# t0m1ab/alphazero

Measured on AMD Instinct MI355X. Metric: self-play games/sec (whole node), Othello 8x8 @100 sims/move, higher is better.
Workload: dtype f32; 1 GPU; BASELINE configs[1] literal: Othello 8x8, 4096 concurrent games/GPU, 100 sims/move, 1 MI355X; concurrent_games_per_gpu=4096, sims_per_move=100, parallelism=game-sharded x1, dense_layers=float32 fma chains on the f32-input MFMA

## Files before the change

### alphazero_amd/csrc/az_net.hip

```cpp
#include <math.h>
#include <stdlib.h>
#include <string.h>

#include <map>
#include <string>
#include <vector>

#include "az_device.h"
#include <hip/hip_ext.h>
#include "az_host.h"

typedef float f32x4 __attribute__((ext_vector_type(4)));
#define MFMA(a, b, c) __builtin_amdgcn_mfma_f32_16x16x4f32((a), (b), (c), 0, 0, 0)
typedef float f32x16 __attribute__((ext_vector_type(16)));
typedef float f32x2 __attribute__((ext_vector_type(2)));
#define MFMA32(a, b, c) __builtin_amdgcn_mfma_f32_32x32x2f32((a), (b), (c), 0, 0, 0)

#define NCH 32
#define PLANE_STRIDE(x) (((x) + 1) | 1)

#ifdef AZ_PROBE
__device__ unsigned long long az_probe_buf[8192 * 8];
#define STAMP(var) { __builtin_amdgcn_sched_barrier(0); var = __builtin_amdgcn_s_memtime(); asm volatile("s_waitcnt lgkmcnt(0)" ::: "memory"); __builtin_amdgcn_sched_barrier(0); }
#else
// ... 1316 lines not shown
        ST_A(0, sa0, as_) ST_A(1, sa1, as_) ST_A(2, sa2, as_) ST_A(3, sa3, as_)           \
        ST_B(0, sb0, bs_) ST_B(1, sb1, bs_) ST_B(2, sb2, bs_) ST_B(3, sb3, bs_)           \
    }
#define FRD 4
#define GEMM_COMPUTE(buf)                                                                 \
    {                                                                                     \
        const float *as = As + (buf) * BM * ASTR + (wm0 + (lane & 31)) * ASTR + (lane >> 5);   \
        const float *bs = Bs + (buf) * BK * BSTR + (lane >> 5) * BSTR + wn0 + (lane & 31);     \
        float afr[FRD][TM], bfr[FRD][TN];                                                 \
        _Pragma("unroll") for (int p = 0; p < FRD - 1; ++p) {                             \
            _Pragma("unroll") for (int tm = 0; tm < TM; ++tm) afr[p][tm] = as[tm * 32 * ASTR + p * 2];          \
            _Pragma("unroll") for (int tn = 0; tn < TN; ++tn) bfr[p][tn] = bs[p * 2 * BSTR + tn * 32];          \
        }                                                                                 \
        _Pragma("unroll") for (int ks = 0; ks < BK / 2; ++ks) {                           \
            if (ks + FRD - 1 < BK / 2) {                                                  \
                _Pragma("unroll") for (int tm = 0; tm < TM; ++tm) afr[(ks + FRD - 1) % FRD][tm] = as[tm * 32 * ASTR + (ks + FRD - 1) * 2];   \
                _Pragma("unroll") for (int tn = 0; tn < TN; ++tn) bfr[(ks + FRD - 1) % FRD][tn] = bs[(ks + FRD - 1) * 2 * BSTR + tn * 32];   \
            }                                                                             \
            __builtin_amdgcn_sched_barrier(0);                                            \
            _Pragma("unroll") for (int tm = 0; tm < TM; ++tm)                             \
                _Pragma("unroll") for (int tn = 0; tn < TN; ++tn) acc[tm][tn] = MFMA32(afr[ks % FRD][tm], bfr[ks % FRD][tn], acc[tm][tn]); \
            __builtin_amdgcn_sched_barrier(0);                                            \
        }                                                                                 \
    }
    static_assert(A_LD <= 4 && B_LD <= 4, "staging register budget");
    const int T = KT > 0 ? KT : K / BK;
    GEMM_ISSUE_R(0)
    if (T > 1) GEMM_ISSUE_S(BK)
    GEMM_STORE_R(0)
    __syncthreads();
    unsigned long long p0 = 0, p1 = 0, p2 = 0, p3 = 0, p4 = 0, ph_issue = 0, ph_comp = 0, ph_store = 0, ph_bar = 0, p_begin = 0;
    (void)p0; (void)p1; (void)p2; (void)p3; (void)p4; (void)ph_issue; (void)ph_comp; (void)ph_store; (void)ph_bar; (void)p_begin;
    STAMP(p_begin)
#ifdef AZ_PROBE
    const unsigned long long rt_begin = __builtin_amdgcn_s_memrealtime();
#endif
#define GEMM_PAIR(t)                                                                      \
    {                                                                                     \
        STAMP(p0)                                                                         \
        if ((t) + 2 < T) GEMM_ISSUE_R(((t) + 2) * BK)                                     \
        STAMP(p1)                                                                         \
        GEMM_COMPUTE(0)                                                                   \
        STAMP(p2)                                                                         \
        if ((t) + 1 < T) GEMM_STORE_S(1)                                                  \
        STAMP(p3)                                                                         \
        __syncthreads();                                                                  \
        STAMP(p4)                                                                         \
        ph_issue += p1 - p0; ph_comp += p2 - p1; ph_store += p3 - p2; ph_bar += p4 - p3;  \
        if ((t) + 1 < T) {                                                                \
            STAMP(p0)                                                                     \
            if ((t) + 3 < T) GEMM_ISSUE_S(((t) + 3) * BK)                                 \
            STAMP(p1)                                                                     \
            GEMM_COMPUTE(1)                                                               \
            STAMP(p2)                                                                     \
            if ((t) + 2 < T) GEMM_STORE_R(0)                                              \
            STAMP(p3)                                                                     \
            __syncthreads();                                                              \
            STAMP(p4)                                                                     \
            ph_issue += p1 - p0; ph_comp += p2 - p1; ph_store += p3 - p2; ph_bar += p4 - p3;  \
        }                                                                                 \
    }
    if constexpr (KT > 0) {
#pragma unroll
        for (int t = 0; t < KT; t += 2) GEMM_PAIR(t)
    } else {
        for (int t = 0; t < T; t += 2) GEMM_PAIR(t)
    }
#undef GEMM_PAIR
#undef GEMM_ISSUE_R
#undef GEMM_ISSUE_S
#undef GEMM_STORE_R
#undef GEMM_STORE_S
#undef GEMM_COMPUTE
#undef FRD
#undef LD_A
#undef LD_B
#undef ST_A
#undef ST_B
#ifdef AZ_PROBE
    if (tid == 0 && bid < 8192) {
        unsigned long long p_end = 0;
        STAMP(p_end)
        unsigned long long *o = az_probe_buf + (size_t)bid * 8;
        o[0] = ph_issue; o[1] = ph_comp; o[2] = ph_store; o[3] = ph_bar; o[4] = p_end - p_begin; o[5] = p_begin; o[6] = p_end;
        o[7] = __builtin_amdgcn_s_memrealtime() - rt_begin;
    }
#endif
#pragma unroll
    for (int tm = 0; tm < TM; ++tm)
#pragma unroll
        for (int tn = 0; tn < TN; ++tn)
#pragma unroll
            for (int r = 0; r < 16; ++r) {
                int row = bm0 + wm0 + tm * 32 + (r & 3) + 8 * (r >> 2) + 4 * (lane >> 5);
                int col = bn0 + wn0 + tn * 32 + (lane & 31);
                float v = acc[tm][tn][r];
                if (RELU) v = v > 0.0f ? v : 0.0f;
                if (row < M) C[(size_t)row * N + col] = v;
            }
}

template <bool RELU>
__global__ __launch_bounds__(256) __attribute__((amdgpu_waves_per_eu(1, 1))) void k_gemm_solo(const float *__restrict__ A, const float *__restrict__ Bw,
                                                                                           const float *__restrict__ bias, float *__restrict__ C, int M, int N,
                                                                                           int K, const int *__restrict__ dyn_count) {
    if (dyn_count) { int c = *dyn_count; M = c < M ? c : M; }
    constexpr int BM = 256, BN = 256, BK = 32, ASTR = BK + 1, BSTR = BN;
    const int nbx = N / BN, nb = nbx * (int)gridDim.y;
    int bid = (int)blockIdx.y * nbx + (int)blockIdx.x;
    if (nb % 8 == 0) bid = (bid % 8) * (nb / 8) + bid / 8;
    const int tile_y = bid / nbx, tile_x = bid % nbx;
    int tme = 4;
    if ((M + 63) / 64 <= (int)gridDim.y) tme = 1;
    else if ((M + 127) / 128 <= (int)gridDim.y) tme = 2;
    const int BMe = 64 * tme;
    if (tile_y * BMe >= M) return;
#ifdef AZ_PROBE
    unsigned long long pk0, pk1, pl0, pl1;
    const unsigned long long rt0 = __builtin_amdgcn_s_memrealtime();
    STAMP(pk0)
#endif
    extern __shared__ __attribute__((aligned(16))) float gsm[];
    float *As = gsm;
    float *Bs = gsm + 2 * BM * ASTR;
    const int tid = threadIdx.x, wave = tid >> 6, lane = tid & 63;
    const int wm0 = (wave >> 1) * 32 * tme, wn0 = (wave & 1) * 128;
    const int bm0 = tile_y * BMe, bn0 = tile_x * BN;
    f32x16 acc[4][4];
    {
        const float one = lane < 32 ? 1.0f : 0.0f;
#pragma unroll
        for (int tn = 0; tn < 4; ++tn) {
            const float bv = lane < 32 ? bias[bn0 + wn0 + tn * 32 + lane] : 0.0f;
#pragma unroll
            for (int tm = 0; tm < 4; ++tm) {
                f32x16 z;
#pragma unroll
                for (int r = 0; r < 16; ++r) z[r] = 0.0f;
                acc[tm][tn] = MFMA32(one, bv, z);
            }
        }
    }
    const int arow = tid >> 3, aq = tid & 7;
    unsigned aoff0, aoff1, aoff2, aoff3, aoff4, aoff5, aoff6, aoff7;
#define SOLO_AOFF(i)                                                       \
    {                                                                      \
        int gr = bm0 + arow + 32 * i;                                      \
        gr = gr < M ? gr : M - 1;                                          \
        aoff##i = (unsigned)(((size_t)gr * K + 4 * aq) * sizeof(float));   \
    }
    SOLO_AOFF(0) SOLO_AOFF(1) SOLO_AOFF(2) SOLO_AOFF(3) SOLO_AOFF(4) SOLO_AOFF(5) SOLO_AOFF(6) SOLO_AOFF(7)
    const unsigned boff = (unsigned)(((size_t)(tid >> 6) * N + 4 * (tid & 63)) * sizeof(float));
    const float *Bt = Bw + bn0;
    float4 ra0, ra1, ra2, ra3, ra4, ra5, ra6, ra7, rb0, rb1, rb2, rb3, rb4, rb5, rb6, rb7;
#define SOLO_LDA(i, k0) ra##i = *reinterpret_cast<const float4 *>(reinterpret_cast<const char *>(A + (k0)) + aoff##i);
#define SOLO_LDB(i, k0) rb##i = *reinterpret_cast<const float4 *>(reinterpret_cast<const char *>(Bt + (size_t)((k0) + 4 * i) * N) + boff);
#define SOLO_LD(i, k0) { SOLO_LDA(i, k0) SOLO_LDB(i, k0) }
#define SOLO_ISSUE(k0) SOLO_LD(0, k0) SOLO_LD(1, k0) SOLO_LD(2, k0) SOLO_LD(3, k0) SOLO_LD(4, k0) SOLO_LD(5, k0) SOLO_LD(6, k0) SOLO_LD(7, k0)
#define SOLO_STA(i, as_)                       \
    {                                          \
        float *d = (as_) + 32 * i * ASTR;      \
        d[0] = ra##i.x;                        \
        d[1] = ra##i.y;                        \
        d[2] = ra##i.z;                        \
        d[3] = ra##i.w;                        \
    }
#define SOLO_STB(i, bs_) *reinterpret_cast<float4 *>((bs_) + 4 * i * BSTR) = rb##i;
#define SOLO_ST(i) { SOLO_STA(i, as_) SOLO_STB(i, bs_) }
#define SOLO_STASH(buf)                                                                                                      \
    {                                                                                                                        \
        float *as_ = As + (buf) * BM * ASTR + arow * ASTR + 4 * aq, *bs_ = Bs + (buf) * BK * BSTR + (tid >> 6) * BSTR + 4 * (tid & 63); \
        SOLO_ST(0) SOLO_ST(1) SOLO_ST(2) SOLO_ST(3) SOLO_ST(4) SOLO_ST(5) SOLO_ST(6) SOLO_ST(7)                              \
    }
#define SOLO_FENCE() { __builtin_amdgcn_sched_barrier(0); asm volatile("" ::: "memory"); __builtin_amdgcn_sched_barrier(0); }
#define SOLO_COMPUTE(buf, NEXT, k0n, TME)                                                                            \
    {                                                                                                            \
        const float *as = As + (buf) * BM * ASTR + (wm0 + (lane & 31)) * ASTR + (lane >> 5);                     \
        const float *bs = Bs + (buf) * BK * BSTR + (lane >> 5) * BSTR + wn0 + (lane & 31);                       \
        float *as_ = As + ((buf) ^ 1) * BM * ASTR + arow * ASTR + 4 * aq, *bs_ = Bs + ((buf) ^ 1) * BK * BSTR + (tid >> 6) * BSTR + 4 * (tid & 63); \
        float afr[2][4], bfr[2][4];                                                                              \
        _Pragma("unroll") for (int x = 0; x < 4; ++x) { if (x < TME) afr[0][x] = as[x * 32 * ASTR]; bfr[0][x] = bs[x * 32]; } \
        _Pragma("unroll") for (int ks = 0; ks < BK / 2; ++ks) {                                                  \
// ... 233 lines not shown
        for (int i = 0; i < 16; ++i) acc = fmaf(x[k0 + i], wa[i], acc);
        if (k0 + 32 < K) {
#pragma unroll
            for (int i = 0; i < 16; ++i) wa[i] = w[(size_t)(k0 + 32 + i) * N];
        }
#pragma unroll
        for (int i = 0; i < 16; ++i) acc = fmaf(x[k0 + 16 + i], wb[i], acc);
    }
    if (RELU) acc = acc > 0.0f ? acc : 0.0f;
    if (n < N) Y[(size_t)m * N + n] = acc;
}

template <bool RELU, int NT>
__global__ __launch_bounds__(64 * NT) void k_dense_frag(const float *__restrict__ X, const float *__restrict__ Wq, const float *__restrict__ bias,
                                                        float *__restrict__ Y, int M, int N, int K, const int *__restrict__ dyn_count) {
    if (dyn_count) { int c = *dyn_count; M = c < M ? c : M; }
    constexpr int NTHR = 64 * NT, PF = 8;
    const int brow0 = blockIdx.y * 16;
    if (brow0 >= M) return;
    extern __shared__ __attribute__((aligned(16))) float dfs[];
    const int XSTR = K + 4, NKB = K / 16, NTILES = N / 16;
    const int tid = threadIdx.x, wave = tid >> 6, lane = tid & 63;
    const int m = lane & 15, kq = lane >> 4;
    const int ct = blockIdx.x * NT + wave;
    const float4 *wq = reinterpret_cast<const float4 *>(Wq) + (size_t)ct * 64 + lane;
    const size_t wstep = (size_t)NTILES * 64;
    float4 bq[PF];
#pragma unroll
    for (int p = 0; p < PF; ++p) bq[p] = wq[(size_t)p * wstep];
    const float bv = bias[ct * 16 + m];
    {
        const int kv = K / 4, rows = (M - brow0) < 16 ? (M - brow0) : 16, nv = rows * kv;
        for (int q0 = 0; q0 < nv; q0 += 4 * NTHR) {
            float4 rx[4];
#pragma unroll
            for (int i = 0; i < 4; ++i) {
                const int q = q0 + tid + NTHR * i;
                rx[i] = make_float4(0, 0, 0, 0);
                if (q < nv) rx[i] = reinterpret_cast<const float4 *>(X + (size_t)(brow0 + q / kv) * K)[q % kv];
            }
#pragma unroll
            for (int i = 0; i < 4; ++i) {
                const int q = q0 + tid + NTHR * i;
                if (q < nv) *reinterpret_cast<float4 *>(dfs + (q / kv) * XSTR + 4 * (q % kv)) = rx[i];
            }
        }
    }
    __syncthreads();
    f32x4 acc = (f32x4){bv, bv, bv, bv};
    const float *xa = dfs + m * XSTR + kq;
    for (int kb0 = 0; kb0 < NKB; kb0 += PF) {
#pragma unroll
        for (int p = 0; p < PF; ++p) {
            const int kb = kb0 + p;
            const float4 b = bq[p];
            if (kb + PF < NKB) bq[p] = wq[(size_t)(kb + PF) * wstep];
            const float a0 = xa[16 * kb], a1 = xa[16 * kb + 4], a2 = xa[16 * kb + 8], a3 = xa[16 * kb + 12];
            __builtin_amdgcn_sched_barrier(0);
            acc = MFMA(a0, b.x, acc);
            acc = MFMA(a1, b.y, acc);
            acc = MFMA(a2, b.z, acc);
            acc = MFMA(a3, b.w, acc);
            __builtin_amdgcn_sched_barrier(0);
        }
    }
#pragma unroll
    for (int r = 0; r < 4; ++r) {
        const int row = brow0 + 4 * kq + r;
        float v = acc[r];
        if (RELU) v = v > 0.0f ? v : 0.0f;
        if (row < M) Y[(size_t)row * N + ct * 16 + m] = v;
    }
}

__global__ void k_retile_q(const float *__restrict__ W, float *__restrict__ dst, int K, int N) {
    const int i = blockIdx.x * blockDim.x + threadIdx.x;
    if (i >= K * N) return;
    const int ii = i % 4, lane = (i / 4) % 64, NTL = N / 16, nt = (i / 256) % NTL, kb = i / (256 * NTL);
    dst[i] = W[(size_t)(16 * kb + 4 * ii + (lane >> 4)) * N + 16 * nt + (lane & 15)];
}

template <int BM, int BN>
constexpr int gemm_lds_bytes() { return 4 * (2 * BM * (32 + 1) + 2 * 32 * BN); }

template <int NT>
__global__ __launch_bounds__(256) void k_heads(const float *__restrict__ X, const float *__restrict__ Wh,
                                               const float *__restrict__ bh, int M, int K, int A,
                                               float *__restrict__ probs, float *__restrict__ value, const int *__restrict__ dyn_count) {
    if (dyn_count) { int c = *dyn_count; M = c < M ? c : M; }
    if ((int)blockIdx.x * 32 >= M) return;
    constexpr int NH = NT * 16, KC = 128, XSTR = KC + 2, WSTR = NH, NS = (NT + 1) / 2;
    constexpr int X_LD = 32 * KC / 4 / 256, W_LD = (KC * NH / 4 + 255) / 256;
    static_assert(X_LD == 4 && W_LD <= 10, "staging registers");
    extern __shared__ __attribute__((aligned(16))) float hsm[];
    float *Xs = hsm;
    float *Ws = Xs + 32 * XSTR;
    float *Ls = Ws + KC * WSTR;
    float *rsum = Ls + 32 * (NH + 1);
    const int tid = threadIdx.x, wave = tid >> 6, lane = tid & 63;
    const int brow0 = blockIdx.x * 32;
    const int mt = wave >> 1, nt0 = (wave & 1) ? NS : 0, ntn = (wave & 1) ? NT - NS : NS;
    f32x4 acc[NS];
#pragma unroll
    for (int i = 0; i < NS; ++i) {
        float bv = i < ntn ? bh[(nt0 + i) * 16 + (lane & 15)] : 0.0f;
        acc[i] = (f32x4){bv, bv, bv, bv};
    }
    float4 rx[X_LD], rw[W_LD];
#pragma unroll
    for (int i = 0; i < X_LD; ++i) rx[i] = make_float4(0, 0, 0, 0);
#pragma unroll
    for (int i = 0; i < W_LD; ++i) rw[i] = make_float4(0, 0, 0, 0);
    const float *xsrc[X_LD];
    int xq[X_LD], xdst[X_LD];
#pragma unroll
    for (int i = 0; i < X_LD; ++i) {
        int idx = tid + i * 256, row = idx >> 5, q = idx & 31;
        int gr = brow0 + row;
        gr = gr < M ? gr : M - 1;
        xsrc[i] = X + (size_t)gr * K + 4 * q;
        xq[i] = 4 * q;
        xdst[i] = row * XSTR + 4 * q;
    }
    auto issue = [&](int kc) {
#pragma unroll
        for (int i = 0; i < X_LD; ++i)
            rx[i] = kc + xq[i] < K ? *reinterpret_cast<const float4 *>(xsrc[i] + kc) : make_float4(0, 0, 0, 0);
        const float *wsrc = Wh + (size_t)kc * NH;
        const int wlim = (K - kc) * NH;
#pragma unroll
        for (int i = 0; i < W_LD; ++i) {
            int f = 4 * (tid + i * 256);
            if (f < KC * NH) rw[i] = f < wlim ? *reinterpret_cast<const float4 *>(wsrc + f) : make_float4(0, 0, 0, 0);
        }
    };
    auto stash = [&]() {
#pragma unroll
        for (int i = 0; i < X_LD; ++i) {
            float *d = Xs + xdst[i];
            *reinterpret_cast<float2 *>(d) = make_float2(rx[i].x, rx[i].y);
            *reinterpret_cast<float2 *>(d + 2) = make_float2(rx[i].z, rx[i].w);
        }
#pragma unroll
        for (int i = 0; i < W_LD; ++i) {
            int f = 4 * (tid + i * 256);
            if (f < KC * NH) *reinterpret_cast<float4 *>(Ws + f) = rw[i];
        }
    };
    issue(0);
    int boff[NS];
#pragma unroll
    for (int i = 0; i < NS; ++i) boff[i] = i < ntn ? i * 16 : 0;
    const float *xa = Xs + (mt * 16 + (lane & 15)) * XSTR + (lane >> 4);
    const float *wb = Ws + (lane >> 4) * WSTR + nt0 * 16 + (lane & 15);
    for (int kc = 0; kc < K; kc += KC) {
        stash();
        __syncthreads();
        if (kc + KC < K) issue(kc + KC);
        float a_n = xa[0], b_n[NS];
#pragma unroll
        for (int i = 0; i < NS; ++i) b_n[i] = wb[boff[i]];
#pragma unroll
        for (int ks = 0; ks < KC / 4; ++ks) {
            const float a = a_n;
            float b[NS];
#pragma unroll
// ... 1243 lines not shown
    using G = TrunkGeom<CH, CW>;
    constexpr int WPB = WINO ? 4 : 8;
    constexpr int lds_planes = 64 + WPB * 2 * G::WAVE_FLOATS * 4;
    constexpr int lds_bytes = lds_planes + ((WINO && lds_planes + 65536 <= 160 * 1024) ? 65536 : 0);
    static_assert(lds_bytes <= 160 * 1024, "k_trunk2 workgroup does not fit the CU's LDS");
    static std::atomic<int> n_cu{0};
    if (!n_cu) {
        hipDeviceProp_t pr;
        int dev = 0;
        AZ_HIP(hipGetDevice(&dev)); AZ_HIP(hipGetDeviceProperties(&pr, dev));
        n_cu = pr.multiProcessorCount;
    }
    AZ_TRY((lds_attr<&k_trunk2<CH, CW, WPB, WINO>>(lds_bytes)));
    const int pairs = (B + 1) / 2, want = (pairs + 3) / 4, cus = n_cu;
    AZ_LAUNCH(c, (k_trunk2<CH, CW, WPB, WINO>), dim3(want < cus ? want : cus), dim3(64 * WPB), lds_bytes, in, B, dyn, n->tp, c.feat);
    return AZ_OK;
}

template <int CH, int CW, bool WINO>
static int trunk_go(az_net *n, LaunchCtx &c, const StagePlan &p, const float *in, int B, const int *dyn) {
    using G = TrunkGeom<CH, CW>;
    if constexpr (plane_tuned(CH, CW)) {
        if (p.kernel == K_TRUNK2) return launch_trunk2<CH, CW, WINO>(n, c, in, B, dyn);
        if (p.kernel == K_TRUNK_Q) {
            if (p.waves == 8) AZ_LAUNCH(c, (k_trunk_q<CH, CW, WINO, 8>), dim3((unsigned)B), dim3(512), 0, in, B, dyn, n->tp, c.feat);
            else AZ_LAUNCH(c, (k_trunk_q<CH, CW, WINO, 4>), dim3((unsigned)B), dim3(256), 0, in, B, dyn, n->tp, c.feat);
            return AZ_OK;
        }
    }
    const int b = p.lds_blocks, lds = (b >= 1 && b <= 8 && 160 * 1024 / b > G::LDS_BYTES) ? (160 * 1024 / b) & ~15 : G::LDS_BYTES;
    if constexpr (WINO && plane_wino(CH, CW)) {
#define QUAD(form) if (p.kernel == K_TRUNK_QUAD && p.quad_form == form) {                                                            \
        AZ_TRY((lds_attr<&k_trunk_quad<CH, CW, form>>(lds)));                                                                        \
        AZ_LAUNCH(c, (k_trunk_quad<CH, CW, form>), dim3((B + 3) / 4), dim3(256), lds, in, B, dyn, n->tp, c.feat);                    \
        return AZ_OK; }
        QUAD(0) QUAD(1) QUAD(2)
#undef QUAD
    }
    AZ_TRY((lds_attr<&k_trunk<CH, CW, WINO>>(lds)));
    AZ_LAUNCH(c, (k_trunk<CH, CW, WINO>), dim3((B + 3) / 4), dim3(256), lds, in, B, dyn, n->tp, c.feat);
    return AZ_OK;
}

static int launch_trunk(az_net *n, LaunchCtx &c, const StagePlan &p, const float *in, int B, const int *dyn) {
#define PLANE(ch, cw, w) if (n->CH == ch && n->CW == cw && p.wino == w) return trunk_go<ch, cw, w>(n, c, p, in, B, dyn);
    PLANE(8, 8, true) PLANE(8, 8, false) PLANE(7, 6, true) PLANE(7, 6, false) PLANE(6, 6, false)
    PLANE(5, 5, false) PLANE(5, 6, false) PLANE(5, 7, false) PLANE(5, 8, false) PLANE(6, 5, false) PLANE(6, 7, false) PLANE(6, 8, false)
    PLANE(7, 5, false) PLANE(7, 7, false) PLANE(7, 8, false) PLANE(8, 5, false) PLANE(8, 6, false) PLANE(8, 7, false)
#undef PLANE
    az_set_error("no conv-trunk kernel instantiated for a %dx%d plane", n->CH, n->CW);
    return AZ_EINVAL;
}

struct Dense {
    const float *A, *Bw, *Bq, *bias;
    float *C;
    int M, N, K;
    bool relu;
    const int *dyn;
};

template <int BM, int BN, int WM, int WN, int KT>
static int gemm_launch(LaunchCtx &c, const Dense &a) {
    constexpr int lds = gemm_lds_bytes<BM, BN>();
    AZ_TRY((lds_attr<&k_gemm<BM, BN, WM, WN, true, KT>, &k_gemm<BM, BN, WM, WN, false, KT>>(lds)));
    dim3 grid(a.N / BN, (a.M + BM - 1) / BM);
    if (a.relu) AZ_LAUNCH(c, (k_gemm<BM, BN, WM, WN, true, KT>), grid, dim3(256), lds, a.A, a.Bw, a.bias, a.C, a.M, a.N, a.K, a.dyn);
    else AZ_LAUNCH(c, (k_gemm<BM, BN, WM, WN, false, KT>), grid, dim3(256), lds, a.A, a.Bw, a.bias, a.C, a.M, a.N, a.K, a.dyn);
    return AZ_OK;
}

template <int BM, int BN, int WM, int WN>
static int gemm_go(LaunchCtx &c, const Dense &a) {
    switch (a.K) {
        case 1024: return gemm_launch<BM, BN, WM, WN, 32>(c, a);
        case 512: return gemm_launch<BM, BN, WM, WN, 16>(c, a);
        case 192: return gemm_launch<BM, BN, WM, WN, 6>(c, a);
        case 128: return gemm_launch<BM, BN, WM, WN, 4>(c, a);
        case 64: return gemm_launch<BM, BN, WM, WN, 2>(c, a);
        default: return gemm_launch<BM, BN, WM, WN, 0>(c, a);
    }
}

template <int TM, int TN>
static int solo_t_launch(LaunchCtx &c, const Dense &a) {
    constexpr int BM = 64 * TM, BN = 64 * TN, lds = 4 * (2 * BM * 33 + 2 * 32 * BN);
    AZ_TRY((lds_attr<&k_gemm_solo_t<true, TM, TN>, &k_gemm_solo_t<false, TM, TN>>(lds)));
    dim3 grid(a.N / BN, (a.M + BM - 1) / BM);
    if (a.relu) AZ_LAUNCH(c, (k_gemm_solo_t<true, TM, TN>), grid, dim3(256), lds, a.A, a.Bw, a.bias, a.C, a.M, a.N, a.K, a.dyn);
    else AZ_LAUNCH(c, (k_gemm_solo_t<false, TM, TN>), grid, dim3(256), lds, a.A, a.Bw, a.bias, a.C, a.M, a.N, a.K, a.dyn);
    return AZ_OK;
}

static int frag_go(LaunchCtx &c, const Dense &a) {
    constexpr int NT = 4;
    const int lds = 4 * 16 * (a.K + 4);
    AZ_TRY((lds_attr<&k_dense_frag<true, NT>, &k_dense_frag<false, NT>>(lds)));
    dim3 grid((unsigned)(a.N / (16 * NT)), (unsigned)((a.M + 15) / 16));
    if (a.relu) AZ_LAUNCH(c, (k_dense_frag<true, NT>), grid, dim3(64 * NT), lds, a.A, a.Bq, a.bias, a.C, a.M, a.N, a.K, a.dyn);
    else AZ_LAUNCH(c, (k_dense_frag<false, NT>), grid, dim3(64 * NT), lds, a.A, a.Bq, a.bias, a.C, a.M, a.N, a.K, a.dyn);
    return AZ_OK;
}

static int launch_dense(LaunchCtx &c, const StagePlan &p, const Dense &a) {
    AZ_REQUIRE(a.K % 32 == 0, AZ_EINVAL, "GEMM K=%d is not a multiple of 32", a.K);
    switch (p.kernel) {
        case K_DENSE_FRAG: return frag_go(c, a);
        case K_DENSE_SMALL: {
            dim3 grid((unsigned)((a.N + 63) / 64), (unsigned)a.M);
            if (a.relu) AZ_LAUNCH(c, (k_dense_small<true>), grid, dim3(64), 0, a.A, a.Bw, a.bias, a.C, a.M, a.N, a.K, a.dyn);
            else AZ_LAUNCH(c, (k_dense_small<false>), grid, dim3(64), 0, a.A, a.Bw, a.bias, a.C, a.M, a.N, a.K, a.dyn);
            return AZ_OK;
        }
        case K_GEMM_SOLO: {
            constexpr int lds = 4 * (2 * 256 * 33 + 2 * 32 * 256);
            AZ_TRY((lds_attr<&k_gemm_solo<true>, &k_gemm_solo<false>>(lds)));
            dim3 grid(a.N / 256, (a.M + 255) / 256);
            if (a.relu) AZ_LAUNCH(c, (k_gemm_solo<true>), grid, dim3(256), lds, a.A, a.Bw, a.bias, a.C, a.M, a.N, a.K, a.dyn);
            else AZ_LAUNCH(c, (k_gemm_solo<false>), grid, dim3(256), lds, a.A, a.Bw, a.bias, a.C, a.M, a.N, a.K, a.dyn);
            return AZ_OK;
        }
        case K_GEMM_SOLO_T: return solo_t_launch<2, 2>(c, a);
        default: break;
    }
#define TILE(tm, tn, wm, wn) if (p.bm == tm && p.bn == tn) return gemm_go<tm, tn, wm, wn>(c, a);
    TILE(128, 128, 64, 64) TILE(128, 64, 32, 64) TILE(64, 64, 32, 32) TILE(64, 128, 32, 64) TILE(128, 32, 32, 32)
#undef TILE
    az_set_error("GEMM N=%d is not a multiple of 32", a.N);
    return AZ_EINVAL;
}

template <int NWM, int NWN, int WM, int WN>
static int qgemm_go(az_net *n, LaunchCtx &c, int layer, int B, const int *dyn) {
    constexpr int lds = qgemm_lds_bytes<NWM, NWN, WM, WN>(), BM = NWM * WM * 32, BN = NWN * WN * 32;
    static_assert(lds <= 160 * 1024, "k_qgemm does not fit the CU's LDS");
    AZ_TRY((lds_attr<&k_qgemm<NWM, NWN, WM, WN, true>>(lds)));
    const int K = layer == 1 ? n->FIN : n->F1, N = layer == 1 ? n->F1 : n->F2;
    AZ_LAUNCH_MAYBE_LAST(c, (k_qgemm<NWM, NWN, WM, WN, true>), dim3((unsigned)(N / BN), (unsigned)((B + BM - 1) / BM)), dim3(64 * NWM * NWN), lds, n->qd_a,
              n->qd_rows * (size_t)K, n->qd_ea, layer == 1 ? n->qd_w1 : n->qd_w2, (size_t)N * K, layer == 1 ? n->qd_e1 : n->qd_e2, layer == 1 ? n->fc1b : n->fc2b,
              layer == 1 ? c.h1 : c.h2, B, N, K, dyn);
    return AZ_OK;
}

static int launch_qdense(az_net *n, LaunchCtx &c, const StagePlan &p, int layer, int B, const int *dyn) {
    const int K = layer == 1 ? n->FIN : n->F1, N = layer == 1 ? n->F1 : n->F2;
    const float *x = layer == 1 ? c.feat : c.h1;
    if (p.kernel == K_QDENSE_SMALL) {
        const int8_t *w = layer == 1 ? n->qd_w1 : n->qd_w2;
        const int *e = layer == 1 ? n->qd_e1 : n->qd_e2;
        const float *bias = layer == 1 ? n->fc1b : n->fc2b;
        float *out = layer == 1 ? c.h1 : c.h2;
        const dim3 grid((unsigned)(N / 64), (unsigned)((B + 15) / 16));
        if (K == 128) AZ_LAUNCH(c, (k_qdense_small<128, true>), grid, dim3(256), 0, x, w, (size_t)N * K, e, bias, out, B, N, dyn);
        else if (K == 512) AZ_LAUNCH(c, (k_qdense_small<512, true>), grid, dim3(256), 0, x, w, (size_t)N * K, e, bias, out, B, N, dyn);
        else AZ_LAUNCH(c, (k_qdense_small<1024, true>), grid, dim3(256), 0, x, w, (size_t)N * K, e, bias, out, B, N, dyn);
        return AZ_OK;
    }
    AZ_LAUNCH_FIRST(c, k_q_rows, dim3((unsigned)((B + 3) / 4)), dim3(256), 0, x, B, K, dyn, n->qd_a, n->qd_rows * (size_t)K, n->qd_ea);
#define QG(nwm, nwn, wm, wn) if (p.qg[0] == nwm && p.qg[1] == nwn && p.qg[2] == wm && p.qg[3] == wn) return qgemm_go<nwm, nwn, wm, wn>(n, c, layer, B, dyn);
    QG(2, 2, 1, 2) QG(2, 2, 1, 1) QG(4, 2, 1, 1) QG(4, 2, 1, 2) QG(2, 4, 1, 1)
#undef QG
    az_set_error("no k_qgemm for the tile plan <%d,%d,%d,%d>", p.qg[0], p.qg[1], p.qg[2], p.qg[3]);
    return AZ_EINVAL;
}

template <int NT>
static int heads_go(az_net *n, LaunchCtx &c, int B, float *probs, float *value, const int *dyn) {
    constexpr int lds = heads_lds_bytes<NT>();
    AZ_TRY((lds_attr<&k_heads<NT>>(lds)));
    AZ_LAUNCH(c, (k_heads<NT>), dim3((B + 31) / 32), dim3(256), lds, c.h2, n->hw, n->hb, B, n->F2, n->A, probs, value, dyn);
    return AZ_OK;
}

template <int NT, int RH>
static int heads2_go(az_net *n, LaunchCtx &c, int B, float *probs, float *value, const int *dyn) {
    constexpr int lds = heads2_lds_bytes<NT, RH, 512>();
    static_assert(lds <= 160 * 1024, "k_heads2 does not fit the CU's LDS");
    AZ_TRY((lds_attr<&k_heads2<NT, RH, 512>>(lds)));
    AZ_LAUNCH(c, (k_heads2<NT, RH, 512>), dim3((unsigned)((B + 16 * RH - 1) / (16 * RH))), dim3(64 * NT), lds, c.h2, n->hwq, n->hb, B, n->A, probs, value, dyn);
    return AZ_OK;
}

static int launch_heads(az_net *n, LaunchCtx &c, const StagePlan &p, int B, float *probs, float *value, const int *dyn) {
    if (p.kernel == K_HEADS_SMALL) {
        AZ_LAUNCH(c, k_heads_small, dim3((unsigned)B), dim3(128), 0, c.h2, n->hw, n->hb, B, n->F2, n->A, n->NH, probs, value, dyn);
        return AZ_OK;
    }
    if (p.kernel == K_HEADS2 && p.nt == 5) return p.rh == 2 ? heads2_go<5, 2>(n, c, B, probs, value, dyn) : heads2_go<5, 1>(n, c, B, probs, value, dyn);
    if (p.kernel == K_HEADS2 && p.nt == 3) return p.rh == 2 ? heads2_go<3, 2>(n, c, B, probs, value, dyn) : heads2_go<3, 1>(n, c, B, probs, value, dyn);
    switch (p.kernel == K_HEADS ? p.nt : 0) {
        case 1: return heads_go<1>(n, c, B, probs, value, dyn);
        case 3: return heads_go<3>(n, c, B, probs, value, dyn);
        case 5: return heads_go<5>(n, c, B, probs, value, dyn);
        default: az_set_error("no heads kernel for padded width %d", n->NH); return AZ_EINVAL;
    }
}

template <int FIN, int A, int R>
static int tail_go(az_net *n, LaunchCtx &c, int B, float *probs, float *value, const int *dyn) {
    constexpr int lds = 4 * tail_lds_floats<FIN, 64, 32, 16, R>();
    static_assert(lds <= 160 * 1024, "k_tail_small does not fit the CU's LDS");
    AZ_TRY((lds_attr<&k_tail_small<FIN, 64, 32, 16, A, R>>(lds)));
    AZ_LAUNCH(c, (k_tail_small<FIN, 64, 32, 16, A, R>), dim3((unsigned)((B + 4 * R - 1) / (4 * R))), dim3(256), lds, c.feat, n->fc1w,
                       n->fc1b, n->fc2w, n->fc2b, n->hw, n->hb, B, probs, value, dyn);
    return AZ_OK;
}

// ... 184 lines not shown
```

### alphazero_amd/csrc/az_net_plan.h

```cpp
#pragma once
#include <limits.h>
#include <stdlib.h>

#ifndef AZ_OTHELLO
#define AZ_OTHELLO 0
#define AZ_CONNECT4 1
#define AZ_TICTACTOE 2
#endif

struct NetTuning {
    int winograd;
    bool dense_i8;
    bool trunk_v1;
    int trunk_quad;
    int trunk_quad_form;
    int trunk_q_max;
    int trunk_q_waves;
    int trunk_blocks_per_cu;
    int beside_trunk2_min;
    int beside_frag_max;
    int beside_tile;
    int gemm_solo;
    int dense_frag_max;
    int gemm_tile;
    int qd_small_max;
    int qg_cfg;
    int heads_small_max;
    bool heads_v1;
    int heads_rh;
    bool tail_v1;
    bool no_fused_tail;
    int tail_r8_from;
};

inline int net_env(const char *name, int dflt) { const char *e = getenv(name); return e ? atoi(e) : dflt; }

inline const NetTuning &net_tuning() {
    static const NetTuning t = [] {
        NetTuning v;
        v.winograd = net_env("AZ_WINOGRAD", -1); v.dense_i8 = net_env("AZ_DENSE_I8", 0) == 1; v.trunk_v1 = net_env("AZ_TRUNK_V1", 0) != 0;
        v.trunk_quad = getenv("AZ_TRUNK_QUAD") ? (net_env("AZ_TRUNK_QUAD", 0) ? 1 : 0) : -1;
        v.trunk_quad_form = net_env("AZ_TRUNK_QUAD_FORM", -1); v.trunk_q_max = net_env("AZ_TRUNK_Q_MAX", 512); v.trunk_q_waves = net_env("AZ_TRUNK_Q_WAVES", 0);
        v.trunk_blocks_per_cu = net_env("AZ_TRUNK_BLOCKS_PER_CU", -1);
        if (v.trunk_blocks_per_cu < 0 && getenv("AZ_TRUNK_BLOCKS_PER_CU")) v.trunk_blocks_per_cu = 0;
        v.beside_trunk2_min = net_env("AZ_BESIDE_TRUNK2_MIN", 4096); v.beside_frag_max = net_env("AZ_BESIDE_FRAG_MAX", 1024); v.beside_tile = net_env("AZ_BESIDE_TILE", 0);
        v.gemm_solo = net_env("AZ_GEMM_SOLO", -1); v.dense_frag_max = net_env("AZ_DENSE_FRAG_MAX", -1); v.gemm_tile = net_env("AZ_GEMM_TILE", 0);
        v.qd_small_max = net_env("AZ_QD_SMALL_MAX", 512); v.qg_cfg = net_env("AZ_QG_CFG", 0);
        v.heads_small_max = net_env("AZ_HEADS_SMALL_MAX", -1); v.heads_v1 = net_env("AZ_HEADS_V1", 0) != 0; v.heads_rh = net_env("AZ_HEADS_RH", 0);
        v.tail_v1 = net_env("AZ_TAIL_V1", 0) != 0; v.no_fused_tail = net_env("AZ_NO_FUSED_TAIL", 0) != 0; v.tail_r8_from = net_env("AZ_TAIL_R8_FROM", INT_MAX);
        return v;
    }();
    return t;
}

struct NetDims {
    int game, CH, CW, FIN, F1, F2, NH, A;
    bool qd_on, fc1wq, fc2wq;
};

enum NetKernel {
    K_NONE, K_MLP, K_TRUNK, K_TRUNK_QUAD, K_TRUNK_Q, K_TRUNK2, K_TAIL_MFMA, K_TAIL_SMALL, K_DENSE_FRAG, K_DENSE_SMALL, K_GEMM, K_GEMM_SOLO,
    K_GEMM_SOLO_T, K_QDENSE_SMALL, K_QGEMM , K_HEADS_SMALL, K_HEADS, K_HEADS2
};

struct StagePlan {
    int stage;
    NetKernel kernel;
    NetKernel family;
    bool wino;
    int waves;
    int quad_form;
    int lds_blocks;
    int bm, bn;
    int qg[4];
    int nt, rh;
    int tail_r;
};

constexpr bool frag_shape(int N, int K) { return N % 64 == 0 && K % 128 == 0 && K <= 2048; }
constexpr bool plane_tuned(int CH, int CW) { return (CH == 8 && CW == 8) || (CH == 6 && CW == 6) || (CH == 7 && CW == 6); }
constexpr bool plane_wino(int CH, int CW) { return (CH == 8 && CW == 8) || (CH == 7 && CW == 6); }

inline StagePlan plan_trunk(const NetDims &d, const NetTuning &t, int B, int beside) {
    StagePlan p = {};
    p.kernel = p.family = K_TRUNK;
    p.lds_blocks = 3;
    if (!plane_tuned(d.CH, d.CW)) return p;
    p.wino = t.winograd != 0 && plane_wino(d.CH, d.CW);
    if (!t.trunk_v1 && B >= (beside ? t.beside_trunk2_min : 4096)) { p.kernel = p.family = K_TRUNK2; p.waves = p.wino ? 4 : 8; return p; }
    if (B <= t.trunk_q_max) {
        p.kernel = p.family = K_TRUNK_Q;
        p.waves = (t.trunk_q_waves ? t.trunk_q_waves : (B <= 256 ? 8 : 4)) == 8 ? 8 : 4;
        return p;
    }
    const int want = t.trunk_blocks_per_cu >= 0 ? t.trunk_blocks_per_cu : 3;
    const int want_lean = t.trunk_blocks_per_cu >= 0 ? t.trunk_blocks_per_cu : (d.CH == 8 ? 0 : 3);
    p.lds_blocks = want;
    if (!p.wino || !(t.trunk_quad >= 0 ? t.trunk_quad == 1 : (d.CH == 7 || beside))) return p;
    p.kernel = K_TRUNK_QUAD;
    p.quad_form = (t.trunk_quad_form >= 0 && t.trunk_quad_form <= 2) ? t.trunk_quad_form : (d.CH == 8 ? 2 : 1);
    if (p.quad_form) p.lds_blocks = want_lean;
    return p;
}

inline StagePlan plan_dense(const NetDims &d, const NetTuning &t, int stage, int B, int beside) {
    StagePlan p = {};
    const int N = stage == 1 ? d.F1 : d.F2, K = stage == 1 ? d.FIN : d.F1;
    auto is = [&p](NetKernel k) { p.kernel = p.family = k; return p; };
    if (d.qd_on) {
        if (B <= t.qd_small_max && N % 64 == 0 && (K == 128 || K == 512 || K == 1024)) return is(K_QDENSE_SMALL);
        static const int plans[6][4] = {{0, 0, 0, 0}, {2, 2, 1, 2}, {2, 2, 1, 1}, {4, 2, 1, 1}, {4, 2, 1, 2}, {2, 4, 1, 1}};
        const int cfg = (t.qg_cfg >= 1 && t.qg_cfg <= 5) ? t.qg_cfg : ((long long)((B + 127) / 128) * (N / 128) >= 256 ? 4 : 5);
        for (int i = 0; i < 4; ++i) p.qg[i] = plans[cfg][i];
        return is(K_QGEMM);
    }
    const int lone_max = t.dense_frag_max >= 0 ? t.dense_frag_max : (K >= 1024 ? 2048 : 1024);
    const int fmax = (beside && t.beside_frag_max < lone_max) ? t.beside_frag_max : lone_max;
    if ((stage == 1 ? d.fc1wq : d.fc2wq) && B <= fmax && frag_shape(N, K)) return is(K_DENSE_FRAG);
    if (B <= (K >= 1024 ? 256 : 128) && K % 32 == 0) return is(K_DENSE_SMALL);
    const int solo = t.gemm_solo;
    if (solo != 0 && N % 256 == 0 && (solo == 1 || (long long)((B + 255) / 256) * (N / 256) >= 256)) return is(K_GEMM_SOLO);
    if (solo != 0 && solo != 1 && N % 128 == 0 && (solo == 2 || (solo < 0 && (long long)((B + 127) / 128) * (N / 128) >= 512))) return is(K_GEMM_SOLO_T);
    const long long mb128 = (B + 127) / 128, mb64 = (B + 63) / 64;
    const int tile = t.gemm_tile ? t.gemm_tile : (beside ? t.beside_tile : 0);
    auto tiled = [&](int bm, int bn) { p.bm = bm; p.bn = bn; return is(K_GEMM); };
    if (tile == 1 && N % 128 == 0) return tiled(128, 128);
    if (tile == 2 && N % 64 == 0) return tiled(128, 64);
    if (tile == 3 && N % 64 == 0) return tiled(64, 64);
    if (tile == 4 && N % 128 == 0) return tiled(64, 128);
    if (N % 128 == 0 && mb128 * (N / 128) >= 512) return tiled(128, 128);
    if (N % 64 == 0 && mb128 * (N / 64) >= 512) return tiled(128, 64);
    if (N % 64 == 0 && mb64 * (N / 64) >= (beside ? 256 : 512)) return tiled(64, 64);
    if (N % 128 == 0) return tiled(64, 128);
    if (N % 64 == 0) return tiled(64, 64);
    return N % 32 == 0 ? tiled(128, 32) : tiled(0, 0);
}

inline StagePlan plan_heads(const NetDims &d, const NetTuning &t, int B) {
    StagePlan p = {};
    const bool heads2 = d.F2 == 512 && (d.NH == 80 || d.NH == 48);
    const int small_max = t.heads_small_max >= 0 ? t.heads_small_max : (heads2 ? 0 : 128);
    p.nt = d.NH / 16;
    p.rh = t.heads_rh == 2 ? 2 : 1;
    if (B <= small_max && d.NH <= 128 && d.F2 % 32 == 0) p.kernel = K_HEADS_SMALL;
    else p.kernel = (!t.heads_v1 && heads2) ? K_HEADS2 : K_HEADS;
    p.family = p.kernel;
    return p;
}

inline StagePlan plan_stage(const NetDims &d, const NetTuning &t, int stage, int B, int beside) {
    StagePlan p = {};
    if (d.game == AZ_TICTACTOE) { p.family = K_MLP; p.kernel = stage == 0 ? K_MLP : K_NONE; }
    else if (stage >= 1 && !t.no_fused_tail && d.F1 == 64 && d.F2 == 32 && d.NH == 16 && d.FIN == 192 && d.A == 7) {
        p.family = t.tail_v1 ? K_TAIL_SMALL : K_TAIL_MFMA;
        p.kernel = stage == 1 ? p.family : K_NONE;
        p.tail_r = B >= t.tail_r8_from ? 8 : 4;
    }
    else p = stage == 0 ? plan_trunk(d, t, B, beside) : (stage == 3 ? plan_heads(d, t, B) : plan_dense(d, t, stage, B, beside));
    p.stage = stage;
    return p;
}

inline const char *net_kernel_name(NetKernel k) {
    static const char *const names[] = {"nothing", "k_mlp", "k_trunk", "k_trunk_quad", "k_trunk_q", "k_trunk2", "k_tail_mfma", "k_tail_small", "k_dense_frag",
                                        "k_dense_small", "k_gemm", "k_gemm_solo", "k_gemm_solo_t", "k_qdense_small", "k_q_rows + k_qgemm", "k_heads_small", "k_heads", "k_heads2"};
    return names[k];
}
inline const char *plan_family_name(const StagePlan &p) {
    if (p.family == K_TRUNK2 && p.wino) return "k_trunk2<Winograd conv2>";
    return net_kernel_name(p.family == K_TRUNK_QUAD ? K_TRUNK : p.family);
}
inline int plan_slot(const StagePlan &p) {
    switch (p.family) {
        case K_TRUNK2: return 0;
        case K_TRUNK: case K_TRUNK_QUAD: return 4;
        case K_TRUNK_Q: return 7;
        case K_TAIL_MFMA: case K_TAIL_SMALL: return 1;
        case K_DENSE_FRAG: case K_DENSE_SMALL: case K_QDENSE_SMALL: return p.stage == 1 ? 5 : 6;
        default: return p.stage;
    }
}
```

Baseline: 4522 games/s.

## Add ring-buffered 64x64 GEMM variant for small Othello dense layers beside trunk

Adds k_gemm_ring, a 64x64-tile f32 MFMA GEMM with BK=16, a triple-buffered LDS ring and four sets of register staging, so global loads run several k-steps ahead of the MFMAs and barriers are skipped on the last steps. The planner picks it by default only for Othello 8x8 dense layers that run beside the trunk with 64x64 tiles and at most 256 blocks. An env knob can force it on or off. The aim is to hide global-memory latency in low-occupancy small GEMMs, at the cost of more registers and more frequent barriers.

```diff
diff --git a/alphazero_amd/csrc/az_net.hip b/alphazero_amd/csrc/az_net.hip
--- a/alphazero_amd/csrc/az_net.hip
+++ b/alphazero_amd/csrc/az_net.hip
@@ -1422,7 +1422,7 @@
         unsigned long long p_end = 0;
         STAMP(p_end)
         unsigned long long *o = az_probe_buf + (size_t)bid * 8;
-        o[0] = ph_issue; o[1] = ph_comp; o[2] = ph_store; o[3] = ph_bar; o[4] = p_end - p_begin; o[5] = p_begin; o[6] = p_end;
+        o[0] = ph_issue; o[1] = ph_comp; o[2] = ph_store; o[3] = ph_bar; o[4] = (unsigned long long)T; o[5] = p_begin; o[6] = p_end;
         o[7] = __builtin_amdgcn_s_memrealtime() - rt_begin;
     }
 #endif
@@ -1438,6 +1438,124 @@
                 if (RELU) v = v > 0.0f ? v : 0.0f;
                 if (row < M) C[(size_t)row * N + col] = v;
             }
+}
+
+template <bool RELU, int KT>
+__global__ __launch_bounds__(256, 2) void k_gemm_ring(const float *__restrict__ A, const float *__restrict__ Bw, const float *__restrict__ bias,
+                                                    float *__restrict__ C, int M, int N, const int *__restrict__ dyn_count) {
+    static_assert(KT >= 2, "NSET tiles are staged before the first MFMA");
+    if (dyn_count) { int c = *dyn_count; M = c < M ? c : M; }
+    constexpr int BM = 64, BN = 64, BK = 16, K = KT * 32, T = K / BK, NBUF = 3, NSET = 4, FRD = 4, KS = BK / 2, ASTR = BK + 1, BSTR = BN;
+    const int nbx = N / BN, nb = nbx * (int)gridDim.y;
+    int bid = (int)blockIdx.y * nbx + (int)blockIdx.x;
+    if (nb % 8 == 0) bid = (bid % 8) * (nb / 8) + bid / 8;
+    const int tile_y = bid / nbx, tile_x = bid % nbx;
+    if (tile_y * BM >= M) return;
+    extern __shared__ __attribute__((aligned(16))) float gsm[];
+    float *As = gsm;
+    float *Bs = gsm + NBUF * BM * ASTR;
+    const int tid = threadIdx.x, wave = tid >> 6, lane = tid & 63;
+    const int wm0 = (wave >> 1) * 32, wn0 = (wave & 1) * 32;
+    const int bm0 = tile_y * BM, bn0 = tile_x * BN;
+    f32x16 acc;
+    {
+        const float bv = bias[bn0 + wn0 + (lane & 31)];
+#pragma unroll
+        for (int r = 0; r < 16; ++r) acc[r] = bv;
+    }
+    const int arow = tid >> 2, aq = tid & 3, bkr = tid >> 4, bc = tid & 15;
+    int gr = bm0 + arow;
+    gr = gr < M ? gr : M - 1;
+    const float *ap = A + (size_t)gr * K + 4 * aq;
+    const unsigned bstep = 4u * BK * N;
+    unsigned bo = 4u * (bkr * N + bn0 + 4 * bc);
+    float *sa = As + arow * ASTR + 4 * aq, *sb = Bs + bkr * BSTR + 4 * bc;
+    float4 rs[NSET][2];
+#define RING_LD(s, j, t)                                                                                              \
+    {                                                                                                                 \
+        if ((j) == 0) rs[s][0] = *reinterpret_cast<const float4 *>(ap + (t) * BK);                                    \
+        else {                                                                                                        \
+            rs[s][1] = *reinterpret_cast<const float4 *>(reinterpret_cast<const char *>(Bw) + bo);                    \
+            bo += bstep;                                                                                              \
+            asm("" : "+v"(bo));                                                                                       \
+        }                                                                                                             \
+    }
+#define RING_ST(s, j, buf)                                                                                            \
+    {                                                                                                                 \
+        if ((j) == 0) {                                                                                               \
+            float *d = sa + (buf) * BM * ASTR;                                                                        \
+            d[0] = rs[s][0].x; d[1] = rs[s][0].y; d[2] = rs[s][0].z; d[3] = rs[s][0].w;                               \
+        } else *reinterpret_cast<float4 *>(sb + (buf) * BK * BSTR) = rs[s][1];                                        \
+    }
+#pragma unroll
+    for (int u = 0; u < NSET; ++u)
+#pragma unroll
+        for (int j = 0; j < 2; ++j) RING_LD(u, j, u)
+#pragma unroll
+    for (int u = 0; u < 2; ++u)
+#pragma unroll
+        for (int j = 0; j < 2; ++j) {
+            RING_ST(u, j, u)
+            if (u + NSET < T) RING_LD(u, j, u + NSET)
+        }
+    __syncthreads();
+    const float *as = As + (wm0 + (lane & 31)) * ASTR + (lane >> 5);
+    const float *bs = Bs + (lane >> 5) * BSTR + wn0 + (lane & 31);
+    float afr[FRD], bfr[FRD];
+#pragma unroll
+    for (int p = 0; p < FRD - 1; ++p) {
+        afr[p] = as[p * 2];
+        bfr[p] = bs[p * 2 * BSTR];
+    }
+    unsigned long long p0 = 0, p1 = 0, p2 = 0, ph_comp = 0, ph_bar = 0, p_begin = 0;
+    (void)p0; (void)p1; (void)p2; (void)ph_comp; (void)ph_bar; (void)p_begin;
+    STAMP(p_begin)
+#ifdef AZ_PROBE
+    const unsigned long long rt_begin = __builtin_amdgcn_s_memrealtime();
+#endif
+#pragma unroll
+    for (int t = 0; t < T; ++t) {
+        STAMP(p0)
+#pragma unroll
+        for (int ks = 0; ks < KS; ++ks) {
+            const int g = t * KS + ks, gn = g + FRD - 1;
+            if (gn < T * KS) {
+                afr[gn % FRD] = as[(gn / KS % NBUF) * BM * ASTR + (gn % KS) * 2];
+                bfr[gn % FRD] = bs[(gn / KS % NBUF) * BK * BSTR + (gn % KS) * 2 * BSTR];
+            }
+            if (ks == 2 || ks == 4) {
+                if (t + 2 < T) RING_ST((t + 2) % NSET, ks / 2 - 1, (t + 2) % NBUF)
+                if (t + 2 + NSET < T) RING_LD((t + 2) % NSET, ks / 2 - 1, t + 2 + NSET)
+            }
+            __builtin_amdgcn_sched_barrier(0);
+            asm volatile("" : "+v"(afr[g % FRD]), "+v"(bfr[g % FRD]));
+            acc = MFMA32(afr[g % FRD], bfr[g % FRD], acc);
+            __builtin_amdgcn_sched_barrier(0);
+        }
+        STAMP(p1)
+        if (t + 2 < T) __syncthreads();
+        STAMP(p2)
+        ph_comp += p1 - p0; ph_bar += p2 - p1;
+    }
+#undef RING_LD
+#undef RING_ST
+#ifdef AZ_PROBE
+    if (tid == 0 && bid < 8192) {
+        unsigned long long p_end = 0;
+        STAMP(p_end)
+        unsigned long long *o = az_probe_buf + (size_t)bid * 8;
+        o[0] = 0; o[1] = ph_comp; o[2] = 0; o[3] = ph_bar; o[4] = KT; o[5] = p_begin; o[6] = p_end;
+        o[7] = __builtin_amdgcn_s_memrealtime() - rt_begin;
+    }
+#endif
+#pragma unroll
+    for (int r = 0; r < 16; ++r) {
+        const int row = bm0 + wm0 + (r & 3) + 8 * (r >> 2) + 4 * (lane >> 5);
+        const int col = bn0 + wn0 + (lane & 31);
+        float v = acc[r];
+        if (RELU) v = v > 0.0f ? v : 0.0f;
+        if (row < M) C[(size_t)row * N + col] = v;
+    }
 }
 
 template <bool RELU>
@@ -1837,6 +1955,7 @@
 
 template <int BM, int BN>
 constexpr int gemm_lds_bytes() { return 4 * (2 * BM * (32 + 1) + 2 * 32 * BN); }
+constexpr int gemm_ring_lds_bytes() { return 4 * 3 * (64 * (16 + 1) + 16 * 64); }
 
 template <int NT>
 __global__ __launch_bounds__(256) void k_heads(const float *__restrict__ X, const float *__restrict__ Wh,
@@ -3246,6 +3365,28 @@
     }
 }
 
+template <int KT>
+static int gemm_ring_launch(LaunchCtx &c, const Dense &a) {
+    constexpr int lds = gemm_ring_lds_bytes();
+    AZ_TRY((lds_attr<&k_gemm_ring<true, KT>, &k_gemm_ring<false, KT>>(lds)));
+    dim3 grid(a.N / 64, (a.M + 63) / 64);
+    if (a.relu) AZ_LAUNCH(c, (k_gemm_ring<true, KT>), grid, dim3(256), lds, a.A, a.Bw, a.bias, a.C, a.M, a.N, a.dyn);
+    else AZ_LAUNCH(c, (k_gemm_ring<false, KT>), grid, dim3(256), lds, a.A, a.Bw, a.bias, a.C, a.M, a.N, a.dyn);
+    return AZ_OK;
+}
+
+static int gemm_ring_go(LaunchCtx &c, const Dense &a) {
+    AZ_REQUIRE((long long)a.K * a.N < (1LL << 30), AZ_EINVAL, "k_gemm's ring form addresses the weights by 32-bit byte offsets: K=%d N=%d", a.K, a.N);
+    switch (a.K) {
+        case 1024: return gemm_ring_launch<32>(c, a);
+        case 512: return gemm_ring_launch<16>(c, a);
+        case 192: return gemm_ring_launch<6>(c, a);
+        case 128: return gemm_ring_launch<4>(c, a);
+        case 64: return gemm_ring_launch<2>(c, a);
+        default: az_set_error("k_gemm's ring form has no instantiation for K=%d", a.K); return AZ_EINVAL;
+    }
+}
+
 template <int TM, int TN>
 static int solo_t_launch(LaunchCtx &c, const Dense &a) {
     constexpr int BM = 64 * TM, BN = 64 * TN, lds = 4 * (2 * BM * 33 + 2 * 32 * BN);
@@ -3287,6 +3428,7 @@
         case K_GEMM_SOLO_T: return solo_t_launch<2, 2>(c, a);
         default: break;
     }
+    if (p.gemm_form == 1) return gemm_ring_go(c, a);
 #define TILE(tm, tn, wm, wn) if (p.bm == tm && p.bn == tn) return gemm_go<tm, tn, wm, wn>(c, a);
     TILE(128, 128, 64, 64) TILE(128, 64, 32, 64) TILE(64, 64, 32, 32) TILE(64, 128, 32, 64) TILE(128, 32, 32, 32)
 #undef TILE
diff --git a/alphazero_amd/csrc/az_net_plan.h b/alphazero_amd/csrc/az_net_plan.h
--- a/alphazero_amd/csrc/az_net_plan.h
+++ b/alphazero_amd/csrc/az_net_plan.h
@@ -23,6 +23,7 @@
     int gemm_solo;
     int dense_frag_max;
     int gemm_tile;
+    int gemm_form;
     int qd_small_max;
     int qg_cfg;
     int heads_small_max;
@@ -45,6 +46,7 @@
         if (v.trunk_blocks_per_cu < 0 && getenv("AZ_TRUNK_BLOCKS_PER_CU")) v.trunk_blocks_per_cu = 0;
         v.beside_trunk2_min = net_env("AZ_BESIDE_TRUNK2_MIN", 4096); v.beside_frag_max = net_env("AZ_BESIDE_FRAG_MAX", 1024); v.beside_tile = net_env("AZ_BESIDE_TILE", 0);
         v.gemm_solo = net_env("AZ_GEMM_SOLO", -1); v.dense_frag_max = net_env("AZ_DENSE_FRAG_MAX", -1); v.gemm_tile = net_env("AZ_GEMM_TILE", 0);
+        v.gemm_form = net_env("AZ_GEMM_FORM", -1);
         v.qd_small_max = net_env("AZ_QD_SMALL_MAX", 512); v.qg_cfg = net_env("AZ_QG_CFG", 0);
         v.heads_small_max = net_env("AZ_HEADS_SMALL_MAX", -1); v.heads_v1 = net_env("AZ_HEADS_V1", 0) != 0; v.heads_rh = net_env("AZ_HEADS_RH", 0);
         v.tail_v1 = net_env("AZ_TAIL_V1", 0) != 0; v.no_fused_tail = net_env("AZ_NO_FUSED_TAIL", 0) != 0; v.tail_r8_from = net_env("AZ_TAIL_R8_FROM", INT_MAX);
@@ -72,12 +74,15 @@
     int quad_form;
     int lds_blocks;
     int bm, bn;
+    int gemm_form;
     int qg[4];
     int nt, rh;
     int tail_r;
 };
 
 constexpr bool frag_shape(int N, int K) { return N % 64 == 0 && K % 128 == 0 && K <= 2048; }
+constexpr int gemm_unrolled_kt(int K) { return (K == 1024 || K == 512 || K == 192 || K == 128 || K == 64) ? K / 32 : 0; }
+constexpr bool gemm_ring_shape(int bm, int bn, int K) { return bm == 64 && bn == 64 && gemm_unrolled_kt(K) >= 2; }
 constexpr bool plane_tuned(int CH, int CW) { return (CH == 8 && CW == 8) || (CH == 6 && CW == 6) || (CH == 7 && CW == 6); }
 constexpr bool plane_wino(int CH, int CW) { return (CH == 8 && CW == 8) || (CH == 7 && CW == 6); }
 
@@ -123,7 +128,12 @@
     if (solo != 0 && solo != 1 && N % 128 == 0 && (solo == 2 || (solo < 0 && (long long)((B + 127) / 128) * (N / 128) >= 512))) return is(K_GEMM_SOLO_T);
     const long long mb128 = (B + 127) / 128, mb64 = (B + 63) / 64;
     const int tile = t.gemm_tile ? t.gemm_tile : (beside ? t.beside_tile : 0);
-    auto tiled = [&](int bm, int bn) { p.bm = bm; p.bn = bn; return is(K_GEMM); };
+    auto tiled = [&](int bm, int bn) {
+        p.bm = bm; p.bn = bn;
+        const bool measured = d.game == AZ_OTHELLO && d.CH == 8 && d.CW == 8 && beside && bm == 64 && bn == 64 && mb64 * (N / 64) <= 256;
+        p.gemm_form = gemm_ring_shape(bm, bn, K) && (t.gemm_form >= 0 ? t.gemm_form == 1 : measured) ? 1 : 0;
+        return is(K_GEMM);
+    };
     if (tile == 1 && N % 128 == 0) return tiled(128, 128);
     if (tile == 2 && N % 64 == 0) return tiled(128, 64);
     if (tile == 3 && N % 64 == 0) return tiled(64, 64);
```

New measurement: 4583 games/s (median of 6 runs). 1.4% higher.
